# pasensio97/SDslam

Hardware: AMD Instinct MI355X
Metric: tracked frames/sec (ORB+ImageAlign+PnP) at 640x480, 1000 kp (higher is better)
Workload: dtype u8; 1 GPU; BASELINE configs[3] at the configs[1] pyramid: 640x480, 8-level x1.2, 1000 kp; ORB extract + ImageAlign (levels 4,3,2) + SearchByProjection + PnP RANSAC (maxIts 200; iterations actually run: tracking.mean_pnp_iterations with --full); pose_solver=pnp, pyramid=8x1.2, unique_scenes=64, inputs=resident in HBM, pose_records=packed on the device every step (single GPU: no collective)

## Files before the change

include/sdslam_hip.h:

```cpp
#ifndef SDSLAM_HIP_H_
#define SDSLAM_HIP_H_

#include <stddef.h>
#include <stdint.h>

#ifdef __cplusplus
extern "C" {
#endif

#define SD_OK 0
#define SD_ERR_INVALID_ARG 1
#define SD_ERR_HIP 2
#define SD_ERR_CAPACITY 3
#define SD_ERR_NO_DEVICE 4
#define SD_FALSE 100

const char* sd_last_error(void);
int sd_device_count(void);
const char* sd_version(void);

int sd_set_option(const char* name, int value);
int sd_get_option(const char* name, int* value);
int sd_option_count(void);
const char* sd_option_name(int index);

typedef struct sd_keypoint {
  float x, y, size, angle, response;
  int32_t octave, class_id;
} sd_keypoint;

typedef struct sd_orb sd_orb;

int sd_orb_create(int nfeatures, float scale_factor, int nlevels, int th_fast,
                  int max_w, int max_h, int max_batch, int device, sd_orb** out);
void sd_orb_destroy(sd_orb* h);

int sd_orb_levels(const sd_orb* h);
int sd_orb_scale_tables(const sd_orb* h, float* sf, float* inv_sf, float* sigma2, float* inv_sigma2);
int sd_orb_features_per_level(const sd_orb* h, int32_t* quota);

int sd_orb_plan_info(int nfeatures, float scale_factor, int nlevels, int th_fast, int w, int hgt,
                     int32_t* level_info , int32_t* cell_zones ,
                     int cell_cap, int32_t* n_cells, uint64_t* bytes_per_frame);

int sd_orb_extract(sd_orb* h, const uint8_t* img, int w, int hgt, int stride,
                   sd_keypoint* kps_out, uint8_t* desc_out, int cap, int* n_out);

int sd_orb_extract_batch(sd_orb* h, const uint8_t* imgs, int n_frames, int w, int hgt, int stride,
                         size_t frame_stride, sd_keypoint* kps_out, uint8_t* desc_out,
                         int cap_per_frame, int32_t* n_out);
int sd_orb_extract_batch_device(sd_orb* h, const void* d_imgs, int n_frames, int w, int hgt,
                                int stride, size_t frame_stride);
int sd_orb_download(sd_orb* h, int frame0, int n_frames, sd_keypoint* kps_out, uint8_t* desc_out,
                    int cap_per_frame, int32_t* n_out);

int sd_orb_set_distortion(sd_orb* h, float fx, float fy, float cx, float cy, float k1, float k2,
                          float p1, float p2, float k3);
int sd_orb_download_undistorted(sd_orb* h, int frame0, int n_frames, sd_keypoint* kps_un_out,
                                int cap_per_frame);

int sd_orb_level_info(const sd_orb* h, int level, int* w, int* hgt);
int sd_orb_level_copy(sd_orb* h, int frame, int level, int padded, uint8_t* out, int out_stride);

int sd_orb_debug_blurred(sd_orb* h, int frame, int level, uint8_t* out, int out_stride);
int sd_orb_debug_cell_counts(sd_orb* h, int frame, int level, int32_t* out, int cap, int* n_cells);
int sd_orb_debug_level_keys(sd_orb* h, int frame, int level, uint32_t* keys_out, int cap, int* n);
int sd_debug_orb_set_keypoints(sd_orb* h, int frame0, int n_frames, const int32_t* n, const sd_keypoint* kps,
                               const uint8_t* desc, int cap);

int sd_orb_set_stream(sd_orb* h, void* hip_stream);
int sd_orb_stream_fence(sd_orb* h, void* hip_stream, int direction);
int sd_orb_sync(sd_orb* h);
int sd_orb_set_profiling(sd_orb* h, int on);
int sd_orb_num_stages(void);
const char* sd_orb_stage_name(int stage);
int sd_orb_stage_ms(sd_orb* h, float* ms_out, int cap);
int sd_orb_stage_bytes(const sd_orb* h, double* bytes_out, int cap);

int sd_dev_alloc(size_t bytes, void** out);
int sd_host_alloc(size_t bytes, void** out);
int sd_host_free(void* p);
int sd_dev_free(void* p);
int sd_dev_upload(void* dst, const void* src, size_t bytes);
int sd_dev_download(void* dst, const void* src, size_t bytes);

typedef struct sd_track sd_track;

int sd_track_create(sd_orb* cur, sd_orb* ref, int max_points, int max_batch, int pnp_max_iterations,
                    sd_track** out);
void sd_track_destroy(sd_track* h);
int sd_track_set_camera(sd_track* h, float fx, float fy, float cx, float cy, float bf,
                        float min_x, float max_x, float min_y, float max_y);
int sd_track_set_last(sd_track* h, int frame0, int n_frames, const int32_t* n_last,
                      const uint8_t* valid, const double* Xw, const uint8_t* desc,
                      const int32_t* octave, const float* angle, const int32_t* obs);
int sd_track_set_poses(sd_track* h, int frame0, int n_frames, const double* Tref_cm,
// ... 239 lines not shown
```

sdslam_amd/__init__.py:

```python
from .capi import (KP_DTYPE, SdError, lib, lib_path, ORBextractor, Tracker, DeviceBuffer, device_count,
                   hamming, plan_info, set_option, get_option, option_names, options)

__all__ = ["KP_DTYPE", "SdError", "lib", "lib_path", "ORBextractor", "Tracker", "DeviceBuffer", "device_count", "hamming", "plan_info",
           "set_option", "get_option", "option_names", "options"]
```

sdslam_amd/capi.py:

```python
import ctypes as C
import os

import numpy as np

_HERE = os.path.dirname(os.path.abspath(__file__))
KP_DTYPE = np.dtype([("x", "<f4"), ("y", "<f4"), ("size", "<f4"), ("angle", "<f4"),
                     ("response", "<f4"), ("octave", "<i4"), ("class_id", "<i4")])
assert KP_DTYPE.itemsize == 28

SD_OK = 0


class SdError(RuntimeError):
    def __init__(self, code, msg):
        super().__init__(f"sdslam_hip status {code}: {msg}")
        self.code = code


def lib_path() -> str:
    return os.environ.get("SD_LIB") or os.path.join(_HERE, "libsdslam_hip.so")


_I, _F, _D, _Z, _P, _S = C.c_int, C.c_float, C.c_double, C.c_size_t, C.c_void_p, C.c_char_p
_PP, _PI = C.POINTER(C.c_void_p), C.POINTER(C.c_int)

_SIGNATURES = {
    "sd_last_error": (_S, []),
    "sd_device_count": (_I, []),
    "sd_version": (_S, []),
    "sd_set_option": (_I, [_S, _I]),
    "sd_get_option": (_I, [_S, _PI]),
    "sd_option_count": (_I, []),
    "sd_option_name": (_S, [_I]),
    "sd_orb_create": (_I, [_I, _F, _I, _I, _I, _I, _I, _I, _PP]),
    "sd_orb_destroy": (None, [_P]),
    "sd_orb_levels": (_I, [_P]),
    "sd_orb_scale_tables": (_I, [_P, _P, _P, _P, _P]),
    "sd_orb_features_per_level": (_I, [_P, _P]),
    "sd_orb_plan_info": (_I, [_I, _F, _I, _I, _I, _I, _P, _P, _I, _P, _P]),
    "sd_orb_extract": (_I, [_P, _P, _I, _I, _I, _P, _P, _I, _P]),
    "sd_orb_extract_batch": (_I, [_P, _P, _I, _I, _I, _I, _Z, _P, _P, _I, _P]),
    "sd_orb_extract_batch_device": (_I, [_P, _P, _I, _I, _I, _I, _Z]),
    "sd_orb_download": (_I, [_P, _I, _I, _P, _P, _I, _P]),
    "sd_orb_set_distortion": (_I, [_P, _F, _F, _F, _F, _F, _F, _F, _F, _F]),
    "sd_orb_download_undistorted": (_I, [_P, _I, _I, _P, _I]),
    "sd_orb_level_info": (_I, [_P, _I, _P, _P]),
    "sd_orb_level_copy": (_I, [_P, _I, _I, _I, _P, _I]),
    "sd_orb_debug_blurred": (_I, [_P, _I, _I, _P, _I]),
    "sd_orb_debug_cell_counts": (_I, [_P, _I, _I, _P, _I, _P]),
    "sd_orb_debug_level_keys": (_I, [_P, _I, _I, _P, _I, _P]),
    "sd_debug_orb_set_keypoints": (_I, [_P, _I, _I, _P, _P, _P, _I]),
    "sd_orb_set_stream": (_I, [_P, _P]),
    "sd_orb_stream_fence": (_I, [_P, _P, _I]),
    "sd_orb_sync": (_I, [_P]),
    "sd_orb_set_profiling": (_I, [_P, _I]),
    "sd_orb_num_stages": (_I, []),
    "sd_orb_stage_name": (_S, [_I]),
    "sd_orb_stage_ms": (_I, [_P, _P, _I]),
    "sd_orb_stage_bytes": (_I, [_P, _P, _I]),
    "sd_dev_alloc": (_I, [_Z, _PP]),
    "sd_host_alloc": (_I, [_Z, _PP]),
    "sd_host_free": (_I, [_P]),
    "sd_dev_free": (_I, [_P]),
    "sd_dev_upload": (_I, [_P, _P, _Z]),
    "sd_dev_download": (_I, [_P, _P, _Z]),
    "sd_track_create": (_I, [_P, _P, _I, _I, _I, _PP]),
    "sd_track_destroy": (None, [_P]),
    "sd_track_set_camera": (_I, [_P, _F, _F, _F, _F, _F, _F, _F, _F, _F]),
    "sd_track_set_last": (_I, [_P, _I, _I, _P, _P, _P, _P, _P, _P, _P]),
    "sd_track_set_poses": (_I, [_P, _I, _I, _P, _P]),
    "sd_track_set_rand": (_I, [_P, _I, _I, _P, _I]),
    "sd_track_set_uright": (_I, [_P, _I, _I, _P, _I]),
    "sd_track_stereo_from_depth": (_I, [_P, _I, _P, _I, _I, _I, _Z]),
    "sd_track_get_stereo": (_I, [_P, _I, _I, _P, _P, _I]),
    "sd_track_stereo_from_depth_device": (_I, [_P, _I, _P, _I, _I, _I, _I, _Z, _F]),
    "sd_track_set_local": (_I, [_P, _I, _I, _P, _P, _P, _P, _P, _P, _P, _P, _P, _P]),
    "sd_track_match_local": (_I, [_P, _I, _F, _F, _F]),
    "sd_track_get_local": (_I, [_P, _I, _I, _P, _I, _P, _P, _P, _P, _P]),
    "sd_track_pose_opt": (_I, [_P, _I, _I]),
    "sd_track_get_pose_opt": (_I, [_P, _I, _I, _P, _P, _I, _P]),
    "sd_track_set_current_broadcast": (_I, [_P, _I]),
    "sd_track_relocalize": (_I, [_P, _I, _I, _F, _I, _I, _I, _P, _P]),
    "sd_track_detect_loop": (_I, [_P, _I, _I, _P, _P, _I, _P, _P, _P]),
    "sd_track_with_motion_model": (_I, [_P, _I, _I, _F, _I, _I, _I]),
    "sd_track_get_tracked": (_I, [_P, _I, _I, _P]),
    "sd_track_local_map": (_I, [_P, _I, _F, _F, _F, _I]),
    "sd_track_get_local_map": (_I, [_P, _I, _I, _P, _I, _P]),
    "sd_track_set_point_flags": (_I, [_P, _I, _I, _P, _P, _I]),
    "sd_track_search_by_points": (_I, [_P, _I, _F, _I]),
    "sd_track_get_point_matches": (_I, [_P, _I, _I, _P, _I, _P]),
    "sd_track_set_sim3_points": (_I, [_P, _I, _I, _P, _P, _I]),
    "sd_track_set_point_matches": (_I, [_P, _I, _I, _P, _I]),
# ... 115 lines not shown
def set_option(name: str, value: int):
    _check(lib().sd_set_option(name.encode(), int(value)))


def get_option(name: str) -> int:
    v = C.c_int(0)
    _check(lib().sd_get_option(name.encode(), C.byref(v)))
    return v.value


def option_names():
    L = lib()
    return [L.sd_option_name(i).decode() for i in range(L.sd_option_count())]


class options:

    def __init__(self, values):
        self.values, self.saved = dict(values), {}

    def __enter__(self):
        for k, v in self.values.items():
            self.saved[k] = get_option(k)
            set_option(k, v)
        return self

    def __exit__(self, *exc):
        for k, v in self.saved.items():
            set_option(k, v)
        return False


def device_count() -> int:
    return int(lib().sd_device_count())


def hamming(a: np.ndarray, b: np.ndarray) -> int:
    a = np.ascontiguousarray(a, np.uint8)
    b = np.ascontiguousarray(b, np.uint8)
    assert a.size == 32 and b.size == 32
    return int(lib().sd_hamming(_p(a), _p(b)))


def plan_info(nfeatures, scale_factor, nlevels, th_fast, w, h):
    lv = np.zeros((nlevels, 8), np.int32)
    zones = np.zeros((65536, 6), np.int32)
    n = C.c_int32()
    nbytes = C.c_uint64()
    _check(lib().sd_orb_plan_info(nfeatures, scale_factor, nlevels, th_fast, w, h, _p(lv), _p(zones), len(zones),
                                  C.byref(n), C.byref(nbytes)))
    return dict(levels=lv, cells=zones[:n.value].copy(), bytes_per_frame=nbytes.value)


def pinned_array(shape, dtype=np.uint8):
    n = int(np.prod(shape)) * np.dtype(dtype).itemsize
    L = lib()
    p = C.c_void_p()
    _check(L.sd_host_alloc(n, C.byref(p)))
    buf = (C.c_uint8 * n).from_address(p.value)
    arr = np.frombuffer(buf, dtype=dtype).reshape(shape)

    class _Owner:
        def __init__(self, ptr):
            self.ptr = ptr

        def __del__(self):
            try:
                L.sd_host_free(self.ptr)
            except Exception:
                pass
    return arr, _Owner(p)


class DeviceBuffer:

    def __init__(self, nbytes: int):
        self.ptr = C.c_void_p()
        self.nbytes = nbytes
        _check(lib().sd_dev_alloc(nbytes, C.byref(self.ptr)))

    def upload(self, arr: np.ndarray):
        arr = np.ascontiguousarray(arr)
        assert arr.nbytes <= self.nbytes
        _check(lib().sd_dev_upload(self.ptr, _p(arr), arr.nbytes))

    def free(self):
        if self.ptr:
            lib().sd_dev_free(self.ptr)
            self.ptr = C.c_void_p()

    def __del__(self):
        try:
            self.free()
        except Exception:
            pass


class ORBextractor:

    def __init__(self, nfeatures=1000, scaleFactor=1.2, nlevels=8, thFAST=20, max_w=640, max_h=480, max_batch=1,
                 device=0):
        self.L = lib()
        self.h = C.c_void_p()
        self.nfeatures, self.nlevels, self.max_batch = nfeatures, nlevels, max_batch
        _check(self.L.sd_orb_create(nfeatures, scaleFactor, nlevels, thFAST, max_w, max_h, max_batch, device,
                                    C.byref(self.h)))
# ... 884 lines not shown
```

sdslam_amd/csrc/orb.hip:

```cpp
#include <hip/hip_runtime.h>

#include <algorithm>
#include <cstring>
#include <string>
#include <vector>

#include "introselect.h"
#include "introselect_wave.h"
#include "orb_internal.h"
#include "sd_sincosf.h"

namespace sd {

#ifndef SD_XCD_REMAP
#define SD_XCD_REMAP 1
#endif
__device__ __forceinline__ void xcd_frame_block(unsigned& frame, unsigned& blk) {
#if SD_XCD_REMAP
  const unsigned nx = gridDim.x, total = nx * gridDim.y;
  const unsigned lin = blockIdx.y * nx + blockIdx.x;
  const unsigned q = total >> 3, r = total & 7u, xcd = lin & 7u;
  const unsigned logical = (xcd < r ? xcd * (q + 1u) : r * (q + 1u) + (xcd - r) * q) + (lin >> 3);
  frame = logical / nx;
  blk = logical - frame * nx;
// ... 243 lines not shown
      const int4 tr = rt[Yr[r]];
      bbv[r] = (uint32_t)tr.z;
      const uint32_t a0 = (uint32_t)(tr.x + base), a1 = (uint32_t)(tr.y + base);
      shv[r] = a0 & 3u;
      const uint32_t* q0 = (const uint32_t*)(sb + (a0 & ~3u));
      const uint32_t* q1 = (const uint32_t*)(sb + (a1 & ~3u));
#pragma unroll
      for (int k = 0; k < 3; k++) {
        u[r][k] = q0[k];
        v[r][k] = q1[k];
      }
    }
#pragma unroll
    for (int r = 0; r < PYR_RPT; r++) {
      const int b0 = (int)(bbv[r] & 0xffff), b1 = (int)(bbv[r] >> 16);
      const unsigned sh = shv[r];
      const uint32_t r0lo = __builtin_amdgcn_alignbyte(u[r][1], u[r][0], sh), r0hi = __builtin_amdgcn_alignbyte(u[r][2], u[r][1], sh);
      const uint32_t r1lo = __builtin_amdgcn_alignbyte(v[r][1], v[r][0], sh), r1hi = __builtin_amdgcn_alignbyte(v[r][2], v[r][1], sh);
      uint32_t pk = 0;
#pragma unroll
      for (int k = 0; k < 4; k++) {
        const us2 w = __builtin_bit_cast(us2, ab[k]);
        const int h0 = (int)__builtin_amdgcn_udot2(__builtin_bit_cast(us2, __builtin_amdgcn_perm(r0hi, r0lo, selP[k])), w, 0u, false);
        const int h1 = (int)__builtin_amdgcn_udot2(__builtin_bit_cast(us2, __builtin_amdgcn_perm(r1hi, r1lo, selP[k])), w, 0u, false);
        const uint32_t ov = (__umulhi((uint32_t)b0 << 12, (uint32_t)h0 & ~15u) + __umulhi((uint32_t)b1 << 12, (uint32_t)h1 & ~15u) + 2u) >> 2;
        pk |= ov << (8 * k);
      }
      packed[r] = pk;
    }
  }
  const int nvalid = L.w + 2 * SD_EDGE - (int)dst_x;
  const uint32_t keep = nvalid >= 4 ? 0xffffffffu : (1u << (8 * nvalid)) - 1u;
#pragma unroll
  for (int r = 0; r < PYR_RPT; r++) {
    if (!live[r]) continue;
    packed[r] &= keep;
    *(uint32_t*)(dstb + (dst_x + (uint32_t)__mul24(PY[r], L.pstride))) = packed[r];
    if (mirror) {
      const int Yi = Yr[r];
      const int prow2 = Yi >= 1 && Yi <= SD_EDGE ? SD_EDGE - Yi : (Yi >= L.h - 20 && Yi <= L.h - 2 ? 2 * L.h + 17 - Yi : -1);
      if (prow2 >= 0) *(uint32_t*)(dstb + (dst_x + (uint32_t)__mul24(prow2, L.pstride))) = packed[r];
    }
  }
}

__global__ __launch_bounds__(256) void k_pyr_split(const LevelGeom L, const LevelGeom S, size_t pyr_frame_bytes, int level,
                                                   const int32_t* __restrict__ coef, const uint8_t* __restrict__ src0, int src_stride,
                                                   size_t src_frame_stride, uint8_t* __restrict__ pyr, int G, unsigned magicG, int Hh,
                                                   int mirror) {
  unsigned uframe, bx;
  xcd_frame_block(uframe, bx);
  pyr_resize_body(L, S, pyr_frame_bytes, level, coef, src0, src_stride, src_frame_stride, pyr, G, magicG, Hh, (int)uframe,
                  bx * 256 + threadIdx.x, mirror);
}

typedef unsigned short fu16;
__device__ __forceinline__ fu16 fmin16(fu16 a, fu16 b) { return a < b ? a : b; }
__device__ __forceinline__ fu16 fmax16(fu16 a, fu16 b) { return a > b ? a : b; }

typedef _Float16 fh2 __attribute__((ext_vector_type(2)));
typedef unsigned short fu2 __attribute__((ext_vector_type(2)));
__device__ __forceinline__ fh2 hmax3(fh2 a, fh2 b, fh2 c) { return __builtin_elementwise_maximum(__builtin_elementwise_maximum(a, b), c); }
__device__ __forceinline__ fh2 hmin3(fh2 a, fh2 b, fh2 c) { return __builtin_elementwise_minimum(__builtin_elementwise_minimum(a, b), c); }
__device__ __forceinline__ fh2 ring_pair(const uint8_t* __restrict__ ca, const uint8_t* __restrict__ cb, int o) {
  const fu2 r = {ca[o], cb[o]};
  return __builtin_bit_cast(fh2, r);
}
__device__ __forceinline__ void fast_ring_score2(const uint8_t* __restrict__ ca, const uint8_t* __restrict__ cb, int tp, int& sa, int& sb) {
  fh2 p[16];
  const int va = ca[0], vb = cb[0];
  p[0] = ring_pair(ca, cb, 3 * tp); p[1] = ring_pair(ca, cb, 3 * tp + 1); p[2] = ring_pair(ca, cb, 2 * tp + 2); p[3] = ring_pair(ca, cb, tp + 3);
  p[4] = ring_pair(ca, cb, 3); p[5] = ring_pair(ca, cb, -tp + 3); p[6] = ring_pair(ca, cb, -2 * tp + 2); p[7] = ring_pair(ca, cb, -3 * tp + 1);
  p[8] = ring_pair(ca, cb, -3 * tp); p[9] = ring_pair(ca, cb, -3 * tp - 1); p[10] = ring_pair(ca, cb, -2 * tp - 2); p[11] = ring_pair(ca, cb, -tp - 3);
  p[12] = ring_pair(ca, cb, -3); p[13] = ring_pair(ca, cb, tp - 3); p[14] = ring_pair(ca, cb, 2 * tp - 2); p[15] = ring_pair(ca, cb, 3 * tp - 1);
  fh2 x3[16], n3[16];
#pragma unroll
  for (int k = 0; k < 16; k++) {
    x3[k] = hmax3(p[k], p[(k + 1) & 15], p[(k + 2) & 15]);
    n3[k] = hmin3(p[k], p[(k + 1) & 15], p[(k + 2) & 15]);
  }
  fh2 x9[16], n9[16];
#pragma unroll
  for (int k = 0; k < 16; k++) {
    x9[k] = hmax3(x3[k], x3[(k + 3) & 15], x3[(k + 6) & 15]);
    n9[k] = hmin3(n3[k], n3[(k + 3) & 15], n3[(k + 6) & 15]);
  }
  fh2 A = hmin3(x9[0], x9[1], x9[2]), B = hmax3(n9[0], n9[1], n9[2]);
#pragma unroll
  for (int k = 3; k < 15; k += 2) {
    A = hmin3(A, x9[k], x9[k + 1]);
    B = hmax3(B, n9[k], n9[k + 1]);
  }
  A = __builtin_elementwise_minimum(A, x9[15]);
  B = __builtin_elementwise_maximum(B, n9[15]);
  const fu2 Au = __builtin_bit_cast(fu2, A), Bu = __builtin_bit_cast(fu2, B);
  sa = max(va - (int)Au.x, (int)Bu.x - va) - 1;
  sb = max(vb - (int)Au.y, (int)Bu.y - vb) - 1;
}

#ifdef SD_PNP_PROF
#define FPROF_FRAMES 256
#define FPROF_CELLS 192
__device__ unsigned long long g_fast_prof_wg[(size_t)FPROF_FRAMES * FPROF_CELLS * 8];
#define FPROF_DECL                                   \
  __shared__ unsigned long long s_fprof[8];          \
  if (threadIdx.x < 8) s_fprof[threadIdx.x] = 0;     \
// ... 728 lines not shown
  const bool fast0_direct = src_aligned && P.lv[0].ncells > 0 && opt(OPT_FAST0_FROM_FRAMES) != 0;
  const int ring_slot = h->ev_calls % sd_orb::kRing;
  bool fast_early = false, pyr_early = false;
  hipStream_t ps = nullptr;
  bool fast_started = false;
  int nfp = 0;

  int mark(StageEvent e, hipStream_t stream) {
    if (prof) SD_HIP_CHECK(hipEventRecord(ev[e], stream));
    return SD_OK;
  }

  int fork() {
    fast_early = frames_ready && !capturing && h->select_recorded && h->stream == h->own_stream && opt(OPT_FAST0_EARLY) != 0;
    if (fast_early) SD_HIP_CHECK(hipStreamWaitEvent(h->fast_stream, h->ev_select_done, 0));
    SD_HIP_CHECK(hipEventRecord(h->ev_body_start, s));
    if (!fast_early) SD_HIP_CHECK(hipStreamWaitEvent(h->fast_stream, h->ev_body_start, 0));
    pyr_early = fast_early && h->nsets == 2 && opt(OPT_PYR_EARLY) != 0;
    ps = pyr_early ? h->aux_stream : s;
    if (pyr_early) SD_HIP_CHECK(hipStreamWaitEvent(ps, h->ev_select_done, 0));
    return mark(EV_PYR_BEGIN, ps);
  }

  int launch_fast(const uint8_t* src, size_t src_frame_stride, const FastSrc& fs, int edge, int first, int ncl, size_t lds, bool wide) {
    if (!fast_started) SD_TRY(mark(EV_FAST_BEGIN, h->fast_stream));
    fast_started = true;
    const bool timed = prof && h->evf_ready && nfp < sd_orb::kFastPairs;
    if (timed) (void)hipEventRecord(h->evf[ring_slot][2 * nfp], h->fast_stream);
    hipLaunchKernelGGL(k_fast_cells, dim3(ncl, n), dim3(256), lds, h->fast_stream, h->d_cells, src, src_frame_stride, fs, edge, h->d_cand,
                       P.cand_per_frame, h->d_cell_count, P.ncells, P.lv[first].cell0, P.thFAST, wide ? 1 : 0);
    if (timed) (void)hipEventRecord(h->evf[ring_slot][2 * nfp + 1], h->fast_stream);
    nfp++;
    return SD_OK;
  }

  int fast_level0_direct() {
    FastSrc fs0;
    memset(&fs0, 0, sizeof(fs0));
    fs0.pstride[0] = stride;
    return launch_fast(d_imgs, frame_stride, fs0, 0, 0, P.lv[0].ncells, hp.fast_lds_level[0], src_wide);
  }

  int pyramid_level(int l) {
    const LevelGeom& L = P.lv[l];
    const LevelGeom& S = P.lv[l > 0 ? l - 1 : 0];
    const bool split = L.w >= 16 && L.fast_resize != 0 && (l > 0 || src_aligned);
    if (!split) {
      dim3 grid((L.pstride + 255) / 256, (L.prows + 4 * PYR_ROWS - 1) / (4 * PYR_ROWS), n), block(64, 4, 1);
      hipLaunchKernelGGL(k_pyr_level, grid, block, 0, ps, L, S, (size_t)P.pyr_frame_bytes, l, d_imgs, stride, frame_stride, h->d_pyr);
      return SD_OK;
    }
    auto magic = [](unsigned d) { return (unsigned)(0xFFFFFFFFull / d) + 1u; };
    const int G = (L.w + 2 * SD_EDGE + 3) / 4;
    const bool mirror = L.h >= 48;
    const int Hh = ((mirror ? L.h : L.prows) + PYR_RPT - 1) / PYR_RPT;
    const unsigned n_resize = (unsigned)(((size_t)Hh * G + 255) / 256);
    hipLaunchKernelGGL(k_pyr_split, dim3(n_resize, n), dim3(256), 0, ps, L, S, (size_t)P.pyr_frame_bytes, l, h->d_coef, d_imgs, stride,
                       frame_stride, h->d_pyr, G, magic((unsigned)G), Hh, mirror ? 1 : 0);
    return SD_OK;
  }

  int fast_of_level(int l, const FastSrc& fsrc) {
    const int merge_from = hp.fast_merge_from;
    const bool merged = l >= merge_from;
    int ncl = P.lv[l].ncells;
    size_t lds = hp.fast_lds_level[l];
    if (merged) {
      if (l != P.nlevels - 1) return SD_OK;
      ncl = 0;
      lds = 0;
      for (int m = merge_from; m < P.nlevels; m++) {
        ncl += P.lv[m].ncells;
        lds = std::max(lds, hp.fast_lds_level[m]);
      }
    }
    if (ncl == 0 || (l == 0 && fast0_direct)) return SD_OK;
    SD_HIP_CHECK(hipEventRecord(h->ev_level[l], ps));
    SD_HIP_CHECK(hipStreamWaitEvent(h->fast_stream, h->ev_level[l], 0));
    return launch_fast(h->d_pyr, (size_t)P.pyr_frame_bytes, fsrc, SD_EDGE, merged ? merge_from : l, ncl, lds, true);
  }

  int blur() {
    SD_HIP_CHECK(hipEventRecord(h->ev_pyr_done, ps));
    SD_HIP_CHECK(hipStreamWaitEvent(h->aux_stream, h->ev_pyr_done, 0));
    if (pyr_early) SD_HIP_CHECK(hipStreamWaitEvent(h->aux_stream, h->ev_body_start, 0));
    SD_TRY(mark(EV_BLUR_BEGIN, h->aux_stream));
    hipLaunchKernelGGL(k_blur, dim3((unsigned)hp.blur_tiles.size(), n), dim3(256), 0, h->aux_stream, h->d_plan, h->d_tiles, h->d_pyr,
                       h->d_blur, h->d_sel_count);
    SD_TRY(mark(EV_BLUR_END, h->aux_stream));
    SD_HIP_CHECK(hipEventRecord(h->ev_blur_done, h->aux_stream));
    return SD_OK;
  }

  int join_fast() {
    if (!fast_started) SD_TRY(mark(EV_FAST_BEGIN, h->fast_stream));
    SD_TRY(mark(EV_FAST_END, h->fast_stream));
    if (prof) h->evf_n[ring_slot] = h->evf_ready ? nfp : 0;
    SD_HIP_CHECK(hipStreamWaitEvent(h->fast_stream, h->ev_pyr_done, 0));
    SD_HIP_CHECK(hipEventRecord(h->ev_fast_done, h->fast_stream));
    SD_HIP_CHECK(hipStreamWaitEvent(s, h->ev_fast_done, 0));
    return SD_OK;
  }

  int select() {
    SD_TRY(mark(EV_SELECT_BEGIN, s));
    const int sel_cap = hp.max_cell_pixels > 12000 ? 1024 : 512;
// ... 154 lines not shown
```

sdslam_amd/csrc/orb_host.hip:

```cpp
#include <hip/hip_runtime.h>

#include <algorithm>
#include <cstring>
#include <string>
#include <vector>

#include "orb_internal.h"

using namespace sd;

static thread_local std::string g_err;
namespace sd {
void set_error(const std::string& msg) { g_err = msg; }
}

static const char* kStageNames[ST_COUNT] = {"pyramid", "fast_nms", "select", "blur", "orient_desc"};

template <class T>
static int dev_alloc(T*& p, size_t count, size_t per = 1) {
  SD_HIP_CHECK(hipMalloc(&p, std::max<size_t>(count, 1) * per * sizeof(T)));
  return SD_OK;
}

template <class T>
// ... 237 lines not shown
  (void)hipSetDevice(h->device);
  if (h->stream) (void)hipStreamSynchronize(h->stream);
  (void)wait_trackers(h);
  orb_drop_graphs(h);
  free_geom(h);
  free_all(fixed_buffers(h));
  for (hipStream_t st : {h->aux_stream, h->fast_stream})
    if (st) { (void)hipStreamSynchronize(st); (void)hipStreamDestroy(st); }
  auto destroy = [](hipEvent_t& e) {
    if (e) (void)hipEventDestroy(e);
  };
  for_each_event(h, destroy);
  for (hipEvent_t& e : h->ev_user_fence) destroy(e);
  for (int r = 0; r < sd_orb::kRing; r++) {
    for (hipEvent_t& e : h->ev[r]) destroy(e);
    for (hipEvent_t& e : h->evf[r]) destroy(e);
  }
  if (h->own_stream) (void)hipStreamDestroy(h->own_stream);
  delete h;
}

int sd_orb_levels(const sd_orb* h) { return h ? h->nlevels : 0; }

int sd_orb_plan_info(int nfeatures, float scale_factor, int nlevels, int th_fast, int w, int hgt, int32_t* level_info,
                     int32_t* cell_zones, int cell_cap, int32_t* n_cells, uint64_t* bytes_per_frame) {
  SD_REQUIRE(level_info && n_cells, SD_ERR_INVALID_ARG, "NULL argument");
  SD_REQUIRE(nfeatures > 0 && nlevels >= 1 && nlevels <= SD_MAX_LEVELS && scale_factor > 1.0f, SD_ERR_INVALID_ARG,
             "bad extractor parameters");
  HostPlan hp;
  plan_tables(nfeatures, scale_factor, nlevels, hp);
  const char* why = "";
  if (!plan_geometry(nfeatures, nlevels, th_fast, w, hgt, hp, &why)) {
    set_error(std::string("unsupported geometry: ") + why);
    return SD_ERR_INVALID_ARG;
  }
  for (int l = 0; l < nlevels; l++) {
    const LevelGeom& L = hp.plan.lv[l];
    int32_t* o = level_info + 8 * l;
    o[0] = L.w; o[1] = L.h; o[2] = L.quota; o[3] = L.cols; o[4] = L.rows; o[5] = L.cellW; o[6] = L.cellH; o[7] = L.nfeaturesCell;
  }
  *n_cells = hp.plan.ncells;
  if (cell_zones) {
    SD_REQUIRE(cell_cap >= hp.plan.ncells, SD_ERR_CAPACITY, "cell_cap too small");
    for (int c = 0; c < hp.plan.ncells; c++) {
      const CellGeom& C = hp.cells[c];
      int32_t* o = cell_zones + 6 * c;
      o[0] = C.level; o[1] = C.zx0; o[2] = C.zy0; o[3] = C.zw; o[4] = C.zh; o[5] = C.evaluated;
    }
  }
  if (bytes_per_frame) *bytes_per_frame = hp.plan.pyr_frame_bytes * 2 + (uint64_t)hp.plan.cand_per_frame * 8;
  return SD_OK;
}

int sd_orb_scale_tables(const sd_orb* h, float* sf, float* inv_sf, float* sigma2, float* inv_sigma2) {
  SD_REQUIRE(h, SD_ERR_INVALID_ARG, "handle is NULL");
  for (int i = 0; i < h->nlevels; i++) {
    if (sf) sf[i] = h->hp.sf[i];
    if (inv_sf) inv_sf[i] = h->hp.inv_sf[i];
    if (sigma2) sigma2[i] = h->hp.sigma2[i];
    if (inv_sigma2) inv_sigma2[i] = h->hp.inv_sigma2[i];
  }
  return SD_OK;
}

int sd_orb_features_per_level(const sd_orb* h, int32_t* quota) {
  SD_REQUIRE(h && quota, SD_ERR_INVALID_ARG, "NULL argument");
  for (int i = 0; i < h->nlevels; i++) quota[i] = h->hp.quota[i];
  return SD_OK;
}

int sd_orb_extract_batch_device(sd_orb* h, const void* d_imgs, int n_frames, int w, int hgt, int stride,
                                size_t frame_stride) {
  SD_REQUIRE(h && d_imgs, SD_ERR_INVALID_ARG, "NULL argument");
  SD_REQUIRE(n_frames >= 1 && n_frames <= h->max_batch, SD_ERR_CAPACITY, "n_frames exceeds max_batch");
  SD_REQUIRE(w >= 1 && hgt >= 1 && stride >= w && frame_stride >= (size_t)stride * (hgt - 1) + w, SD_ERR_INVALID_ARG,
             "bad image shape/stride");
  SD_HIP_CHECK(hipSetDevice(h->device));
  return extract_device(h, (const uint8_t*)d_imgs, n_frames, w, hgt, stride, frame_stride, true);
}

int sd_orb_download(sd_orb* h, int frame0, int n_frames, sd_keypoint* kps_out, uint8_t* desc_out, int cap_per_frame,
                    int32_t* n_out) {
  SD_REQUIRE(h && n_out, SD_ERR_INVALID_ARG, "NULL argument");
  SD_TRY(check_frame_range(h, frame0, n_frames));
  SD_TRY(download_counts(h, frame0, n_frames, cap_per_frame, !kps_out && !desc_out, n_out));
  const int cap = std::max(h->hp.plan.nsel, 1);
  if (cap_per_frame == cap && n_frames > 8) {
    if (kps_out)
      SD_HIP_CHECK(hipMemcpyAsync(kps_out, h->d_kps + (size_t)frame0 * cap, (size_t)n_frames * cap * sizeof(sd_keypoint),
                                  hipMemcpyDeviceToHost, h->stream));
    if (desc_out)
      SD_HIP_CHECK(hipMemcpyAsync(desc_out, h->d_desc + (size_t)frame0 * cap * 32, (size_t)n_frames * cap * 32, hipMemcpyDeviceToHost,
                                  h->stream));
  } else {
    if (kps_out) SD_TRY(download_rows(h, h->d_kps, sizeof(sd_keypoint), kps_out, frame0, n_frames, cap_per_frame, n_out));
    if (desc_out) SD_TRY(download_rows(h, h->d_desc, 32, desc_out, frame0, n_frames, cap_per_frame, n_out));
  }
  SD_HIP_CHECK(hipStreamSynchronize(h->stream));
  return SD_OK;
}

int sd_orb_extract_batch(sd_orb* h, const uint8_t* imgs, int n_frames, int w, int hgt, int stride, size_t frame_stride,
                         sd_keypoint* kps_out, uint8_t* desc_out, int cap_per_frame, int32_t* n_out) {
  SD_REQUIRE(h && n_out, SD_ERR_INVALID_ARG, "NULL argument");
  if (w <= 0 || hgt <= 0 || !imgs) {
    for (int f = 0; f < n_frames; f++) n_out[f] = 0;
// ... 250 lines not shown
```

sdslam_amd/csrc/orb_plan.cpp:

```cpp
#include "orb_plan.h"
#include "sd_common.h"

#include <algorithm>
#include <cfloat>
#include <cmath>
#include <cstdlib>
#include <cstring>

namespace sd {

static inline int cv_round(float v) { return (int)lrintf(v); }
static inline int cv_round(double v) { return (int)lrint(v); }
static inline int cv_floor(double v) { int i = (int)v; return i - (i > v); }
static inline size_t up(size_t v, size_t a) { return (v + a - 1) / a * a; }

void plan_tables(int nfeatures, float scaleFactorArg, int nlevels, HostPlan& hp) {
  const double scaleFactor = scaleFactorArg;
  hp.sf.assign(nlevels, 1.0f);
  hp.sigma2.assign(nlevels, 1.0f);
  for (int i = 1; i < nlevels; i++) {
    hp.sf[i] = (float)(hp.sf[i - 1] * scaleFactor);
    hp.sigma2[i] = hp.sf[i] * hp.sf[i];
  }
  hp.inv_sf.resize(nlevels);
// ... 25 lines not shown
    f -= s;
    if (clamp_x) {
      if (s < 0) { f = 0; s = 0; }
      if (s + 1 >= sn && s >= sn - 1) { f = 0; s = sn - 1; }
    }
    float c0 = 1.f - f, c1 = f;
    int a0 = std::min(std::max(cv_round(c0 * 2048.f), -32768), 32767);
    int a1 = std::min(std::max(cv_round(c1 * 2048.f), -32768), 32767);
    ofs[d] = s;
    ab[d] = (int32_t)((uint32_t)(uint16_t)(int16_t)a0 | ((uint32_t)(uint16_t)(int16_t)a1 << 16));
  }
}

static bool group_table(LevelGeom& L, int src_w, const std::vector<int32_t>* xo, const std::vector<int32_t>* xa, std::vector<int32_t>& coef) {
  while (coef.size() % 4) coef.push_back(0);
  L.cg = (int)coef.size();
  auto refl = [](int p, int len) {
    if (len == 1) return 0;
    while (p < 0 || p >= len) p = p < 0 ? -p : 2 * len - 2 - p;
    return p;
  };
  bool ok = true;
  const int G = (L.w + 2 * SD_EDGE + 3) / 4;
  for (int gi = 0; gi < G; gi++) {
    int Xr[4], sx[4] = {0, 0, 0, 0};
    uint32_t ab[4] = {0, 0, 0, 0}, selP[4] = {0, 0, 0, 0};
    for (int k = 0; k < 4; k++) Xr[k] = refl(4 * gi - SD_EDGE + k, L.w);
    int base = 0;
    if (xo) {
      for (int k = 0; k < 4; k++) {
        sx[k] = (*xo)[Xr[k]];
        ab[k] = (uint32_t)(*xa)[Xr[k]];
      }
      base = std::min(std::min(sx[0], sx[1]), std::min(sx[2], sx[3]));
      for (int k = 0; k < 4; k++) {
        const int o = sx[k] - base, o1 = std::min(sx[k] + 1, src_w - 1) - base;
        if (o < 0 || o > 7 || o1 < 0 || o1 > 7) ok = false;
        selP[k] = (uint32_t)o | 0x0c00u | ((uint32_t)o1 << 16) | 0x0c000000u;
      }
    }
    const int Xmin = std::min(std::min(Xr[0], Xr[1]), std::min(Xr[2], Xr[3]));
    uint32_t sel0 = 0;
    for (int k = 0; k < 4; k++) {
      if (Xr[k] - Xmin > 3) ok = false;
      sel0 |= (uint32_t)((Xr[k] - Xmin) & 3) << (8 * k);
    }
    const int32_t e[12] = {base, (int32_t)selP[0], (int32_t)selP[1], (int32_t)selP[2], (int32_t)selP[3], (int32_t)ab[0], (int32_t)ab[1],
                           (int32_t)ab[2], (int32_t)ab[3], Xmin, (int32_t)sel0, 0};
    coef.insert(coef.end(), e, e + 12);
  }
  return ok;
}

bool plan_geometry(int nfeatures, int nlevels, int thFAST, int w, int h, HostPlan& hp, const char** why) {
  (void)nfeatures;
  if (nlevels < 1 || nlevels > SD_MAX_LEVELS) { *why = "nlevels out of range"; return false; }
  if (w < 1 || h < 1 || w > SD_MAX_DIM || h > SD_MAX_DIM) { *why = "image size out of range (1..4095)"; return false; }
  OrbPlan& P = hp.plan;
  memset(&P, 0, sizeof(P));
  P.nlevels = nlevels;
  P.thFAST = std::min(std::max(thFAST, 0), 255);
  P.w0 = w;
  P.h0 = h;
  hp.cells.clear();
  hp.blur_tiles.clear();
  hp.coef.clear();
  hp.max_cells_per_level = 0;
  hp.max_cell_pixels = 0;

  size_t off = 0;
  uint32_t cand = 0;
  int sel = 0;
  const float imageRatio = (float)w / h;
  size_t lds_max = 0;
  {
    hp.fast_merge_from = std::max(1, opt(OPT_FAST_MERGE_FROM));
  }
  for (int l = 0; l < SD_MAX_LEVELS; l++) hp.fast_lds_level[l] = 0;
  double sum_px = 0, px0 = 0, px_last = 0;

  for (int l = 0; l < nlevels; l++) {
    LevelGeom& L = P.lv[l];
    float scale = hp.inv_sf[l];
    L.w = cv_round((float)w * scale);
    L.h = cv_round((float)h * scale);
    if (L.w < 1 || L.h < 1) { *why = "pyramid level collapses to zero size"; return false; }
    L.pstride = (int)up((size_t)L.w + 2 * SD_EDGE, 64);
    L.prows = L.h + 2 * SD_EDGE;
    L.off = (uint32_t)off;
    off += up((size_t)L.pstride * L.prows, 256);
    L.quota = hp.quota[l];
    L.scale = hp.sf[l];
    L.kpsize = (float)(int)(31 * hp.sf[l]);
    L.sel_off = sel;
    sel += L.quota;
    sum_px += (double)L.w * L.h;
    if (l == 0) px0 = (double)L.w * L.h;
    px_last = (double)L.w * L.h;

    L.area2x2 = 0;
    L.fast_resize = 0;
    L.cx = L.cy = L.cg = L.cr = 0;
    L.scale_x = L.scale_y = 1.0;
    if (l > 0) {
      const LevelGeom& S = P.lv[l - 1];
      double sx = 1. / ((double)L.w / S.w), sy = 1. / ((double)L.h / S.h);
      L.scale_x = sx;
      L.scale_y = sy;
      int isx = cv_round(sx), isy = cv_round(sy);
      bool fast = std::fabs(sx - isx) < DBL_EPSILON && std::fabs(sy - isy) < DBL_EPSILON;
      if (fast && isx == 2 && isy == 2) {
        L.area2x2 = 1;
      } else {
        std::vector<int32_t> xo, xa, yo, yb;
        resize_tables(S.w, L.w, xo, xa, true);
        resize_tables(S.h, L.h, yo, yb, false);
        L.cx = (int)hp.coef.size();
        hp.coef.insert(hp.coef.end(), xo.begin(), xo.end());
        hp.coef.insert(hp.coef.end(), xa.begin(), xa.end());
        L.cy = (int)hp.coef.size();
        hp.coef.insert(hp.coef.end(), yo.begin(), yo.end());
        hp.coef.insert(hp.coef.end(), yb.begin(), yb.end());
        bool ok = L.w >= 8;
        for (int x0 = 0; ok && x0 + 3 < L.w; x0++)
          if (std::min(xo[x0 + 3] + 1, S.w - 1) - xo[x0] > 7 || xo[x0 + 3] < xo[x0]) ok = false;
        for (int x = 0; ok && x < L.w; x++)
          if ((xa[x] & 0xffff) > 2048 || ((uint32_t)xa[x] >> 16) > 2048) ok = false;
        for (int y = 0; ok && y < L.h; y++)
          if (yo[y] < 0 || (yb[y] & 0xffff) > 2048 || ((uint32_t)yb[y] >> 16) > 2048) ok = false;
        L.fast_resize = ok ? 1 : 0;
        if (ok) ok = group_table(L, S.w, &xo, &xa, hp.coef);
        if (ok) {
          while (hp.coef.size() % 4) hp.coef.push_back(0);
          L.cr = (int)hp.coef.size();
          for (int y = 0; y < L.h; y++) {
            const int sy0 = std::min(yo[y], S.h - 1), sy1 = std::min(yo[y] + 1, S.h - 1);
            hp.coef.push_back((sy0 + SD_EDGE) * S.pstride + SD_EDGE);
            hp.coef.push_back((sy1 + SD_EDGE) * S.pstride + SD_EDGE);
            hp.coef.push_back(yb[y]);
            hp.coef.push_back(0);
          }
        }
        L.fast_resize = ok ? 1 : 0;
      }
    } else {
      L.fast_resize = group_table(L, 0, nullptr, nullptr, hp.coef) ? 1 : 0;
    }

    const int nDesired = L.quota;
    const int levelCols = (int)sqrtf((float)nDesired / (5 * imageRatio));
    const int levelRows = (int)(imageRatio * levelCols);
    L.cell0 = (int)hp.cells.size();
    L.cand_off = cand;
    L.cols = L.rows = L.ncells = 0;
    L.cellW = L.cellH = L.nfeaturesCell = 0;
    if (levelCols > 0 && levelRows > 0 && nDesired > 0) {
      const int minBX = SD_EDGE, minBY = SD_EDGE, maxBX = L.w - SD_EDGE, maxBY = L.h - SD_EDGE;
      const int W = maxBX - minBX, H = maxBY - minBY;
      const int cellW = (int)ceilf((float)W / levelCols);
      const int cellH = (int)ceilf((float)H / levelRows);
      L.cols = levelCols;
      L.rows = levelRows;
      L.cellW = cellW;
      L.cellH = cellH;
      L.ncells = levelCols * levelRows;
      L.nfeaturesCell = (int)ceilf((float)nDesired / L.ncells);
      for (int i = 0; i < levelRows; i++) {
        const int iniY = minBY + i * cellH - 3;
        int hY = cellH + 6;
        if (i == levelRows - 1) hY = maxBY + 3 - iniY;
        for (int j = 0; j < levelCols; j++) {
          const int iniX = minBX + j * cellW - 3;
          int hX = cellW + 6;
          if (j == levelCols - 1) hX = maxBX + 3 - iniX;
          CellGeom c;
          c.level = l;
          bool skip = (i == levelRows - 1 && hY <= 0) || (j == levelCols - 1 && hX <= 0) || iniX < 0 ||
                      iniY < 0 || hX < 0 || hY < 0 || iniX + hX > L.w || iniY + hY > L.h;
          bool ok = !skip && hX > 6 && hY > 6;
          c.evaluated = skip ? 0 : 1;
          c.zx0 = iniX + 3;
          c.zy0 = iniY + 3;
          c.zw = ok ? hX - 6 : 0;
          c.zh = ok ? hY - 6 : 0;
          if (c.zw == 1) { *why = "a grid cell's FAST zone is one pixel wide (frame too small for this many features per level)"; return false; }
          c.cap = ok ? (uint32_t)(((c.zw + 1) / 2) * ((c.zh + 1) / 2)) : 0;
          c.cand_off = cand;
          cand += c.cap;
          c.strip_rows = 0;
          if (ok) hp.max_cell_pixels = std::max(hp.max_cell_pixels, c.zw * c.zh);
          if (ok) {
            const size_t lds_kb = (size_t)opt(OPT_FAST_LDS_KB);
            const size_t whole_kb = (size_t)opt(OPT_FAST_LDS_WHOLE_KB);
            int S = c.zh;
// ... 56 lines not shown
```

sdslam_amd/csrc/orb_plan.h:

```cpp
#pragma once
#include <stdint.h>
#include <vector>

#define SD_MAX_LEVELS 16
#define SD_EDGE 19
#define SD_MAX_DIM 4095

namespace sd {

struct LevelGeom {
  int w, h;
  int pstride;
  int prows;
  uint32_t off;
  int quota;
  int cols, rows;
  int cellW, cellH;
  int nfeaturesCell;
  int cell0, ncells;
  int sel_off;
  int area2x2;
  int cx, cy;
  int cr;
  int cg;
  int fast_resize;
  double scale_x, scale_y;
  float scale;
  float kpsize;
  uint32_t cand_off;
  uint32_t cand_cap;
};

struct CellGeom {
  int level;
  int zx0, zy0, zw, zh;
  uint32_t cand_off;
  uint32_t cap;
  int strip_rows;
  int evaluated;
};

struct BlurTile { int level, p0, nstrips; unsigned magic; };

struct OrbPlan {
  int nlevels, ncells, nsel;
  int thFAST;
  int w0, h0;
  uint32_t cand_per_frame;
  uint64_t pyr_frame_bytes;
  LevelGeom lv[SD_MAX_LEVELS];
};

struct HostPlan {
  OrbPlan plan;
  std::vector<CellGeom> cells;
  std::vector<BlurTile> blur_tiles;
  std::vector<int32_t> coef;
  std::vector<float> sf, inv_sf, sigma2, inv_sigma2;
  std::vector<int> quota;
  size_t fast_lds_bytes;
  int fast_merge_from;
  size_t fast_lds_level[SD_MAX_LEVELS];
  int max_cells_per_level;
  int max_cell_pixels;
  double stage_bytes[8];
};

void plan_tables(int nfeatures, float scaleFactor, int nlevels, HostPlan& hp);
bool plan_geometry(int nfeatures, int nlevels, int thFAST, int w, int h, HostPlan& hp, const char** why);

}
```

sdslam_amd/csrc/sd_common.h:

```cpp
#pragma once
#include <hip/hip_runtime.h>
#include <stdint.h>
#include <stdio.h>
#include <string>

#include "../../include/sdslam_hip.h"

namespace sd {

void set_error(const std::string& msg);

#define SD_HIP_CHECK(expr)                                                              \
  do {                                                                                  \
    hipError_t _e = (expr);                                                             \
    if (_e != hipSuccess) {                                                             \
      ::sd::set_error(std::string(#expr) + ": " + hipGetErrorString(_e) + " (" + __FILE__ + \
                      ":" + std::to_string(__LINE__) + ")");                            \
      return SD_ERR_HIP;                                                                \
    }                                                                                   \
  } while (0)

#define SD_REQUIRE(cond, code, msg) \
  do {                              \
    if (!(cond)) {                  \
      ::sd::set_error(msg);         \
      return (code);                \
    }                               \
  } while (0)

#define SD_TRY(call) do { const int _rc = (call); if (_rc != SD_OK) return _rc; } while (0)

enum Opt {
  OPT_FAST0_FROM_FRAMES, OPT_USE_GRAPH, OPT_SELECT_SMALL_CAP, OPT_SELECT_BIG_CAP, OPT_FAST_MERGE_FROM, OPT_FAST_LDS_KB,
  OPT_FAST_LDS_WHOLE_KB, OPT_TRACK_PRIORITY, OPT_ALIGN_START, OPT_ALIGN_MIN_WAVES, OPT_BF_LIST_K,
  OPT_POSEOPT_WAVES, OPT_MATCH_SPLIT, OPT_FAST0_EARLY, OPT_PYR_EARLY, OPT_COUNT
};
int opt(Opt o);

static inline size_t align_up(size_t v, size_t a) { return (v + a - 1) / a * a; }

}
```

sdslam_amd/csrc/sd_options.cpp:

```cpp
#include <atomic>
#include <cstring>

#include "sd_common.h"

namespace sd {

struct OptDef {
  const char* name;
  int def, lo, hi;
};

static const OptDef kOpts[OPT_COUNT] = {
    {"extract.fast0_from_frames", 1, 0, 1},
    {"extract.use_graph", 0, 0, 1},
    {"extract.select_small_cap", 0, 0, 1 << 20},
    {"extract.select_big_cap", 0, 0, 1 << 20},
    {"extract.fast_merge_from", 6, 1, 64},
    {"extract.fast_lds_kb", 24, 4, 160},
    {"extract.fast_lds_whole_kb", 40, 4, 160},
    {"track.stream_priority", 2, 0, 2},
    {"track.align_start", 2, 0, 2},
    {"track.align_min_waves", 5, 3, 5},
    {"track.bf_list_k", 4, 1, 4},
    {"track.poseopt_waves", 0, 0, 4},
    {"track.match_split", 1, 0, 1},
    {"extract.fast0_early", 1, 0, 1},
    {"extract.pyr_early", 0, 0, 1},
};

static std::atomic<int> g_val[OPT_COUNT];
static std::atomic<bool> g_init{false};

static void init_once() {
  if (g_init.load(std::memory_order_acquire)) return;
  static std::atomic_flag busy = ATOMIC_FLAG_INIT;
  while (busy.test_and_set(std::memory_order_acquire)) {}
  if (!g_init.load(std::memory_order_relaxed)) {
    for (int i = 0; i < OPT_COUNT; i++) g_val[i].store(kOpts[i].def, std::memory_order_relaxed);
    g_init.store(true, std::memory_order_release);
  }
  busy.clear(std::memory_order_release);
}

int opt(Opt o) {
  init_once();
  return g_val[o].load(std::memory_order_relaxed);
}

}

using namespace sd;

extern "C" {

int sd_set_option(const char* name, int value) {
  SD_REQUIRE(name, SD_ERR_INVALID_ARG, "option name is NULL");
  init_once();
  for (int i = 0; i < OPT_COUNT; i++)
    if (std::strcmp(name, kOpts[i].name) == 0) {
      SD_REQUIRE(value >= kOpts[i].lo && value <= kOpts[i].hi, SD_ERR_INVALID_ARG, std::string("value out of range for option ") + name);
      g_val[i].store(value, std::memory_order_relaxed);
      return SD_OK;
    }
  set_error(std::string("unknown option: ") + name);
  return SD_ERR_INVALID_ARG;
}

int sd_get_option(const char* name, int* value) {
  SD_REQUIRE(name && value, SD_ERR_INVALID_ARG, "NULL argument");
  init_once();
  for (int i = 0; i < OPT_COUNT; i++)
    if (std::strcmp(name, kOpts[i].name) == 0) {
      *value = g_val[i].load(std::memory_order_relaxed);
      return SD_OK;
    }
  set_error(std::string("unknown option: ") + name);
  return SD_ERR_INVALID_ARG;
}

int sd_option_count(void) { return OPT_COUNT; }
// ... 4 lines not shown
```

Before: 241,500 frames/s.

## Add row-block pyramid resize kernel that reuses source rows across consecutive output rows

```diff
diff --git a/include/sdslam_hip.h b/include/sdslam_hip.h
--- a/include/sdslam_hip.h
+++ b/include/sdslam_hip.h
@@ -42,6 +42,9 @@
 int sd_orb_plan_info(int nfeatures, float scale_factor, int nlevels, int th_fast, int w, int hgt,
                      int32_t* level_info , int32_t* cell_zones ,
                      int cell_cap, int32_t* n_cells, uint64_t* bytes_per_frame);
+
+int sd_orb_plan_row_blocks(int nfeatures, float scale_factor, int nlevels, int th_fast, int w, int hgt, int level,
+                           int32_t* blocks , int block_cap, int32_t* n_blocks);
 
 int sd_orb_extract(sd_orb* h, const uint8_t* img, int w, int hgt, int stride,
                    sd_keypoint* kps_out, uint8_t* desc_out, int cap, int* n_out);
diff --git a/sdslam_amd/__init__.py b/sdslam_amd/__init__.py
--- a/sdslam_amd/__init__.py
+++ b/sdslam_amd/__init__.py
@@ -1,5 +1,5 @@
 from .capi import (KP_DTYPE, SdError, lib, lib_path, ORBextractor, Tracker, DeviceBuffer, device_count,
-                   hamming, plan_info, set_option, get_option, option_names, options)
+                   hamming, plan_info, plan_row_blocks, set_option, get_option, option_names, options)
 
-__all__ = ["KP_DTYPE", "SdError", "lib", "lib_path", "ORBextractor", "Tracker", "DeviceBuffer", "device_count", "hamming", "plan_info",
+__all__ = ["KP_DTYPE", "SdError", "lib", "lib_path", "ORBextractor", "Tracker", "DeviceBuffer", "device_count", "hamming", "plan_info", "plan_row_blocks",
            "set_option", "get_option", "option_names", "options"]
diff --git a/sdslam_amd/capi.py b/sdslam_amd/capi.py
--- a/sdslam_amd/capi.py
+++ b/sdslam_amd/capi.py
@@ -38,6 +38,7 @@
     "sd_orb_scale_tables": (_I, [_P, _P, _P, _P, _P]),
     "sd_orb_features_per_level": (_I, [_P, _P]),
     "sd_orb_plan_info": (_I, [_I, _F, _I, _I, _I, _I, _P, _P, _I, _P, _P]),
+    "sd_orb_plan_row_blocks": (_I, [_I, _F, _I, _I, _I, _I, _I, _P, _I, _P]),
     "sd_orb_extract": (_I, [_P, _P, _I, _I, _I, _P, _P, _I, _P]),
     "sd_orb_extract_batch": (_I, [_P, _P, _I, _I, _I, _I, _Z, _P, _P, _I, _P]),
     "sd_orb_extract_batch_device": (_I, [_P, _P, _I, _I, _I, _I, _Z]),
@@ -259,6 +260,13 @@
     return dict(levels=lv, cells=zones[:n.value].copy(), bytes_per_frame=nbytes.value)
 
 
+def plan_row_blocks(nfeatures, scale_factor, nlevels, th_fast, w, h, level):
+    out = np.zeros((4096, 4), np.int32)
+    n = C.c_int32()
+    _check(lib().sd_orb_plan_row_blocks(nfeatures, scale_factor, nlevels, th_fast, w, h, level, _p(out), len(out), C.byref(n)))
+    return out[:n.value].copy()
+
+
 def pinned_array(shape, dtype=np.uint8):
     n = int(np.prod(shape)) * np.dtype(dtype).itemsize
     L = lib()
diff --git a/sdslam_amd/csrc/orb.hip b/sdslam_amd/csrc/orb.hip
--- a/sdslam_amd/csrc/orb.hip
+++ b/sdslam_amd/csrc/orb.hip
@@ -319,6 +319,69 @@
   xcd_frame_block(uframe, bx);
   pyr_resize_body(L, S, pyr_frame_bytes, level, coef, src0, src_stride, src_frame_stride, pyr, G, magicG, Hh, (int)uframe,
                   bx * 256 + threadIdx.x, mirror);
+}
+
+__global__ __launch_bounds__(256) void k_pyr_rows(const LevelGeom L, const LevelGeom S, size_t pyr_frame_bytes,
+                                                  const int32_t* __restrict__ coef, uint8_t* __restrict__ pyr, int G, unsigned magicG) {
+  constexpr int R = SD_PYR_BLOCK_ROWS;
+  unsigned uframe, bx;
+  xcd_frame_block(uframe, bx);
+  const unsigned e = bx * 256 + threadIdx.x;
+  const unsigned bi = __umulhi(e, magicG);
+  if (bi >= (unsigned)L.nblk) return;
+  const int gi = (int)(e - bi * (unsigned)G);
+  const int4* gt = (const int4*)(coef + L.cg) + 3 * gi;
+  const int4* bt = (const int4*)(coef + L.cb) + 2 * bi;
+  const int4 t0 = gt[0], t1 = gt[1], t2 = gt[2];
+  const int4 k0 = bt[0], k1 = bt[1];
+  typedef unsigned short us2 __attribute__((ext_vector_type(2)));
+  const uint32_t selP[4] = {(uint32_t)t0.y, (uint32_t)t0.z, (uint32_t)t0.w, (uint32_t)t1.x};
+  const uint32_t ab[4] = {(uint32_t)t1.y, (uint32_t)t1.z, (uint32_t)t1.w, (uint32_t)t2.x};
+  const uint32_t bb[R] = {(uint32_t)k0.w, (uint32_t)k1.x, (uint32_t)k1.y, (uint32_t)k1.z, (uint32_t)k1.w};
+  const int y0 = k0.x, n = k0.y & 0xff, sy0 = k0.z;
+  const uint8_t* sb = pyr + (size_t)uframe * pyr_frame_bytes + S.off;
+  uint8_t* dstb = pyr + (size_t)uframe * pyr_frame_bytes + L.off;
+  const uint32_t c0 = (uint32_t)(SD_EDGE * S.pstride + SD_EDGE + t0.x);
+  const unsigned sh = c0 & 3u;
+  uint32_t u[R + 1][3];
+#pragma unroll
+  for (int j = 0; j <= R; j++) {
+    const uint32_t* q = (const uint32_t*)(sb + ((c0 & ~3u) + (uint32_t)__mul24(min(sy0 + j, S.h - 1), S.pstride)));
+#pragma unroll
+    for (int k = 0; k < 3; k++) u[j][k] = q[k];
+  }
+  uint32_t hz[R + 1][4];
+#pragma unroll
+  for (int j = 0; j <= R; j++) {
+    const uint32_t lo = __builtin_amdgcn_alignbyte(u[j][1], u[j][0], sh), hi = __builtin_amdgcn_alignbyte(u[j][2], u[j][1], sh);
+#pragma unroll
+    for (int k = 0; k < 4; k++)
+      hz[j][k] = __builtin_amdgcn_udot2(__builtin_bit_cast(us2, __builtin_amdgcn_perm(hi, lo, selP[k])), __builtin_bit_cast(us2, ab[k]), 0u, false) & ~15u;
+  }
+  const uint32_t dst_x = 4u * (uint32_t)gi;
+  const int nvalid = L.w + 2 * SD_EDGE - (int)dst_x;
+  const uint32_t keep = nvalid >= 4 ? 0xffffffffu : (1u << (8 * nvalid)) - 1u;
+  uint32_t packed[R];
+#pragma unroll
+  for (int r = 0; r < R; r++) {
+    const uint32_t b0 = (bb[r] & 0xffffu) << 12, b1 = bb[r] >> 16 << 12;
+    uint32_t pk = 0;
+#pragma unroll
+    for (int k = 0; k < 4; k++)
+      pk |= ((__umulhi(b0, hz[r][k]) + __umulhi(b1, hz[r + 1][k]) + 2u) >> 2) << (8 * k);
+    packed[r] = pk & keep;
+  }
+#pragma unroll
+  for (int r = 0; r < R; r++)
+    if (r < n) *(uint32_t*)(dstb + (dst_x + (uint32_t)__mul24(y0 + r + SD_EDGE, L.pstride))) = packed[r];
+  if (k0.y >> 8) {
+#pragma unroll
+    for (int r = 0; r < R; r++) {
+      const int Yi = y0 + r;
+      const int prow2 = Yi >= 1 && Yi <= SD_EDGE ? SD_EDGE - Yi : (Yi >= L.h - 20 && Yi <= L.h - 2 ? 2 * L.h + 17 - Yi : -1);
+      if (r < n && prow2 >= 0) *(uint32_t*)(dstb + (dst_x + (uint32_t)__mul24(prow2, L.pstride))) = packed[r];
+    }
+  }
 }
 
 typedef unsigned short fu16;
@@ -1153,6 +1216,12 @@
     }
     auto magic = [](unsigned d) { return (unsigned)(0xFFFFFFFFull / d) + 1u; };
     const int G = (L.w + 2 * SD_EDGE + 3) / 4;
+    if (l > 0 && L.nblk > 0) {
+      const unsigned n_rows = (unsigned)(((size_t)L.nblk * G + 255) / 256);
+      hipLaunchKernelGGL(k_pyr_rows, dim3(n_rows, n), dim3(256), 0, ps, L, S, (size_t)P.pyr_frame_bytes, h->d_coef, h->d_pyr, G,
+                         magic((unsigned)G));
+      return SD_OK;
+    }
     const bool mirror = L.h >= 48;
     const int Hh = ((mirror ? L.h : L.prows) + PYR_RPT - 1) / PYR_RPT;
     const unsigned n_resize = (unsigned)(((size_t)Hh * G + 255) / 256);
diff --git a/sdslam_amd/csrc/orb_host.hip b/sdslam_amd/csrc/orb_host.hip
--- a/sdslam_amd/csrc/orb_host.hip
+++ b/sdslam_amd/csrc/orb_host.hip
@@ -313,6 +313,32 @@
   return SD_OK;
 }
 
+int sd_orb_plan_row_blocks(int nfeatures, float scale_factor, int nlevels, int th_fast, int w, int hgt, int level, int32_t* blocks,
+                           int block_cap, int32_t* n_blocks) {
+  SD_REQUIRE(n_blocks, SD_ERR_INVALID_ARG, "NULL argument");
+  SD_REQUIRE(nfeatures > 0 && nlevels >= 1 && nlevels <= SD_MAX_LEVELS && scale_factor > 1.0f && level >= 0 && level < nlevels,
+             SD_ERR_INVALID_ARG, "bad extractor parameters");
+  HostPlan hp;
+  plan_tables(nfeatures, scale_factor, nlevels, hp);
+  const char* why = "";
+  if (!plan_geometry(nfeatures, nlevels, th_fast, w, hgt, hp, &why)) {
+    set_error(std::string("unsupported geometry: ") + why);
+    return SD_ERR_INVALID_ARG;
+  }
+  const LevelGeom& L = hp.plan.lv[level];
+  *n_blocks = L.nblk;
+  if (blocks) {
+    SD_REQUIRE(block_cap >= L.nblk, SD_ERR_CAPACITY, "block_cap too small");
+    for (int b = 0; b < L.nblk; b++) {
+      PyrRowBlock k;
+      memcpy(&k, hp.coef.data() + L.cb + (size_t)b * (sizeof(PyrRowBlock) / 4), sizeof(k));
+      int32_t* o = blocks + 4 * b;
+      o[0] = k.y0; o[1] = k.n_border & 0xff; o[2] = k.sy0; o[3] = k.n_border >> 8;
+    }
+  }
+  return SD_OK;
+}
+
 int sd_orb_scale_tables(const sd_orb* h, float* sf, float* inv_sf, float* sigma2, float* inv_sigma2) {
   SD_REQUIRE(h, SD_ERR_INVALID_ARG, "handle is NULL");
   for (int i = 0; i < h->nlevels; i++) {
diff --git a/sdslam_amd/csrc/orb_plan.cpp b/sdslam_amd/csrc/orb_plan.cpp
--- a/sdslam_amd/csrc/orb_plan.cpp
+++ b/sdslam_amd/csrc/orb_plan.cpp
@@ -101,6 +101,31 @@
   return ok;
 }
 
+static void row_blocks(LevelGeom& L, const std::vector<int32_t>& yo, const std::vector<int32_t>& yb, int mode,
+                       std::vector<int32_t>& coef) {
+  if (mode == 0 || L.h < 48) return;
+  std::vector<PyrRowBlock> blocks;
+  for (int y0 = 0; y0 < L.h;) {
+    int n = 1;
+    while (n < SD_PYR_BLOCK_ROWS && y0 + n < L.h && yo[y0 + n] == yo[y0 + n - 1] + 1) n++;
+    PyrRowBlock b;
+    memset(&b, 0, sizeof(b));
+    b.y0 = y0;
+    b.sy0 = yo[y0];
+    const bool border = (y0 <= SD_EDGE && y0 + n - 1 >= 1) || (y0 <= L.h - 2 && y0 + n - 1 >= L.h - 20);
+    b.n_border = n | (border ? 1 << 8 : 0);
+    for (int r = 0; r < SD_PYR_BLOCK_ROWS; r++) b.bb[r] = (uint32_t)yb[std::min(y0 + r, L.h - 1)];
+    blocks.push_back(b);
+    y0 += n;
+  }
+  if (mode == 1 && (size_t)L.h * 5 < blocks.size() * SD_PYR_BLOCK_ROWS * 4) return;
+  while (coef.size() % 4) coef.push_back(0);
+  L.cb = (int)coef.size();
+  L.nblk = (int)blocks.size();
+  const int32_t* p = (const int32_t*)blocks.data();
+  coef.insert(coef.end(), p, p + blocks.size() * (sizeof(PyrRowBlock) / 4));
+}
+
 bool plan_geometry(int nfeatures, int nlevels, int thFAST, int w, int h, HostPlan& hp, const char** why) {
   (void)nfeatures;
   if (nlevels < 1 || nlevels > SD_MAX_LEVELS) { *why = "nlevels out of range"; return false; }
@@ -149,7 +174,7 @@
 
     L.area2x2 = 0;
     L.fast_resize = 0;
-    L.cx = L.cy = L.cg = L.cr = 0;
+    L.cx = L.cy = L.cg = L.cr = L.cb = L.nblk = 0;
     L.scale_x = L.scale_y = 1.0;
     if (l > 0) {
       const LevelGeom& S = P.lv[l - 1];
@@ -189,6 +214,7 @@
             hp.coef.push_back(yb[y]);
             hp.coef.push_back(0);
           }
+          row_blocks(L, yo, yb, opt(OPT_PYR_ROWS), hp.coef);
         }
         L.fast_resize = ok ? 1 : 0;
       }
diff --git a/sdslam_amd/csrc/orb_plan.h b/sdslam_amd/csrc/orb_plan.h
--- a/sdslam_amd/csrc/orb_plan.h
+++ b/sdslam_amd/csrc/orb_plan.h
@@ -23,6 +23,7 @@
   int cx, cy;
   int cr;
   int cg;
+  int cb, nblk;
   int fast_resize;
   double scale_x, scale_y;
   float scale;
@@ -39,6 +40,15 @@
   int strip_rows;
   int evaluated;
 };
+
+#define SD_PYR_BLOCK_ROWS 5
+struct PyrRowBlock {
+  int32_t y0;
+  int32_t n_border;
+  int32_t sy0;
+  uint32_t bb[SD_PYR_BLOCK_ROWS];
+};
+static_assert(sizeof(PyrRowBlock) == 32, "k_pyr_rows reads a block as two 16-byte loads");
 
 struct BlurTile { int level, p0, nstrips; unsigned magic; };
 
diff --git a/sdslam_amd/csrc/sd_common.h b/sdslam_amd/csrc/sd_common.h
--- a/sdslam_amd/csrc/sd_common.h
+++ b/sdslam_amd/csrc/sd_common.h
@@ -33,7 +33,7 @@
 enum Opt {
   OPT_FAST0_FROM_FRAMES, OPT_USE_GRAPH, OPT_SELECT_SMALL_CAP, OPT_SELECT_BIG_CAP, OPT_FAST_MERGE_FROM, OPT_FAST_LDS_KB,
   OPT_FAST_LDS_WHOLE_KB, OPT_TRACK_PRIORITY, OPT_ALIGN_START, OPT_ALIGN_MIN_WAVES, OPT_BF_LIST_K,
-  OPT_POSEOPT_WAVES, OPT_MATCH_SPLIT, OPT_FAST0_EARLY, OPT_PYR_EARLY, OPT_COUNT
+  OPT_POSEOPT_WAVES, OPT_MATCH_SPLIT, OPT_FAST0_EARLY, OPT_PYR_EARLY, OPT_PYR_ROWS, OPT_COUNT
 };
 int opt(Opt o);
 
diff --git a/sdslam_amd/csrc/sd_options.cpp b/sdslam_amd/csrc/sd_options.cpp
--- a/sdslam_amd/csrc/sd_options.cpp
+++ b/sdslam_amd/csrc/sd_options.cpp
@@ -26,6 +26,7 @@
     {"track.match_split", 1, 0, 1},
     {"extract.fast0_early", 1, 0, 1},
     {"extract.pyr_early", 0, 0, 1},
+    {"extract.pyr_rows", 1, 0, 2},
 };
 
 static std::atomic<int> g_val[OPT_COUNT];
```

New measurement: 248,600 frames/s (median of 6 runs). +3.0%, better.
